# cts198859/deeprl_signal_control

Measured on AMD Instinct MI355X. Metric: env-steps/s (agents x envs x sim-steps/s), large_grid MA2C, higher is better.
Workload: dtype f32; 1 GPU; large_grid 5x5 (25 agents), MA2C LSTM policy (neighbour fingerprint gather), 1024 env instances per GPU; step = 120 control steps (x5 sim-steps) of every instance + 1 A2C update (BPTT, clip, RMSProp); envs_per_gpu=1024, n_step=120, agents=25, parallelism=env-sharded x1, live_vehicles=window mean over the timed region

## Files before the change

deeprl_signal_control_amd/csrc/tsc_model.hip:

```cpp
#include "tsc_common.h"
#include "tsc_gemm.h"
#include "../../include/tsc.h"

#include <cstdlib>
#include <type_traits>
#include <vector>

namespace {

using tsc::f32x16;
using tsc::f32x4;
using tsc::GemmArgs;

constexpr int kOut = 8;
constexpr int kL = 64;
constexpr int kG4 = 4 * kL;

struct Layout {
    int G, A, SMAX, AMAX, H;
    int NZ, fc;
    long long stride, oW1, ob1, oWx, oWh, obl, oWo, obo;
};

__device__ __forceinline__ float sigmoidf_(float x) {
// ... 103 lines not shown
            if (e < E) {
                const long long n = (long long)g * N + (long long)t * E + e;
                if (store) {
                    Z[n * kG4 + j] = ig; Z[n * kG4 + 64 + j] = fg; Z[n * kG4 + 128 + j] = og; Z[n * kG4 + 192 + j] = ug;
                    Cc[n * kL + j] = cn;
                }
                Hh[n * kL + j] = hn;
                if (t + 1 < T) keep = 1.0f - (float)done[(long long)(t + 1) * E + e];
                if (t + 1 == T && state_out) {
                    float *s = state_out + ((long long)g * E + e) * 2 * kL;
                    s[j] = cn; s[kL + j] = hn;
                }
            }
            c[r] = cn * keep;
            hs[j * kHsLd + erow[r]] = hn * keep;
        }
        __syncthreads();
    }
}

constexpr int kDz2Ld = kG4 + 4;
constexpr int kDh3Ld = kL + 4;

__global__ void __launch_bounds__(256, 2) lstm_bwd2_kernel(const float *__restrict__ params, Layout lay, float *Z,
                                                            const float *Cc, const float *state_bw, const float *dH,
                                                            const uint8_t *done, int T, int E) {
    extern __shared__ __attribute__((aligned(16))) char smem_raw[];
    float *dzs = (float *)smem_raw;
    float *dhs = dzs + 32 * kDz2Ld;
    const int g = blockIdx.x, e0 = blockIdx.y * 32;
    const int tid = threadIdx.x, lane = tid & 63, wave = tid >> 6, n = lane & 15, kq = lane >> 4;
    const int j = 16 * wave + n;
    const int er = tid >> 3, u0 = (tid & 7) * 8;
    const long long N = (long long)T * E;
    float bw[64];
    {
        const float4 *src = reinterpret_cast<const float4 *>(params + (long long)g * lay.stride + lay.oWh + (long long)j * kG4 + 4 * kq);
#pragma unroll
        for (int q = 0; q < 16; ++q) {
            const float4 w4 = src[4 * q];
            bw[4 * q] = w4.x; bw[4 * q + 1] = w4.y; bw[4 * q + 2] = w4.z; bw[4 * q + 3] = w4.w;
        }
    }
    float dc_rec[8];
#pragma unroll
    for (int r = 0; r < 8; ++r) dc_rec[r] = 0.f;
    const float *zg = Z + (long long)g * N * kG4, *cg = Cc + (long long)g * N * kL, *hg = dH + (long long)g * N * kL;
    const float *sg = state_bw + (long long)g * E * 2 * kL;
    const int e = e0 + er < E ? e0 + er : E - 1;
    const bool live = e0 + er < E;
    struct In { float4 gi[2], gf[2], go[2], gu[2], dhi[2], cpv[2]; float keep; };
    In in0, in1;
    float4 cc[2];
    auto request = [&](int t, In &o) {
        const long long nt = (long long)t * E;
        const float *zt = zg + nt * kG4, *ct = cg + nt * kL, *ht = hg + nt * kL;
        const float *cp_base = t > 0 ? ct - (long long)E * kL : sg;
        const unsigned cp_ld = t > 0 ? kL : 2 * kL;
        int zq = 0;
        asm volatile("" : "+v"(zq));
        const unsigned oz = (unsigned)((e + zq) * kG4 + u0) * 4u, oc = (unsigned)((e + zq) * kL + u0) * 4u;
#pragma unroll
        for (int a = 0; a < 2; ++a) {
            o.gi[a] = ldg((const float4 *)zt, oz + 16u * a); o.gf[a] = ldg((const float4 *)zt, oz + 256u + 16u * a);
            o.go[a] = ldg((const float4 *)zt, oz + 512u + 16u * a); o.gu[a] = ldg((const float4 *)zt, oz + 768u + 16u * a);
            o.dhi[a] = ldg((const float4 *)ht, oc + 16u * a);
            o.cpv[a] = ldg((const float4 *)cp_base, (unsigned)((e + zq) * cp_ld + u0) * 4u + 16u * a);
        }
        o.keep = done[nt + e] == 0 ? 1.0f : 0.0f;
    };
    {
        const float *ct = cg + (long long)(T - 1) * E * kL;
        cc[0] = ldg((const float4 *)ct, (unsigned)(e * kL + u0) * 4u); cc[1] = ldg((const float4 *)ct, (unsigned)(e * kL + u0) * 4u + 16u);
    }
    request(T - 1, in0);
    if (T > 1) request(T - 2, in1);
    float keep_next = 0.f;
    auto step = [&](int t, In &cur) {
        const long long nt = (long long)t * E;
        float *zw = Z + ((long long)g * N + nt) * kG4;
        const float keep = cur.keep;
        float4 dhr[2];
        if (t == T - 1) { dhr[0] = dhr[1] = make_float4(0.f, 0.f, 0.f, 0.f); }
        else {
            dhr[0] = *reinterpret_cast<const float4 *>(dhs + er * kDh3Ld + u0);
            dhr[1] = *reinterpret_cast<const float4 *>(dhs + er * kDh3Ld + u0 + 4);
        }
#pragma unroll
        for (int a = 0; a < 2; ++a) {
            const float igv[4] = {cur.gi[a].x, cur.gi[a].y, cur.gi[a].z, cur.gi[a].w}, fgv[4] = {cur.gf[a].x, cur.gf[a].y, cur.gf[a].z, cur.gf[a].w};
            const float ogv[4] = {cur.go[a].x, cur.go[a].y, cur.go[a].z, cur.go[a].w}, ugv[4] = {cur.gu[a].x, cur.gu[a].y, cur.gu[a].z, cur.gu[a].w};
            const float ccv[4] = {cc[a].x, cc[a].y, cc[a].z, cc[a].w}, cpw[4] = {cur.cpv[a].x, cur.cpv[a].y, cur.cpv[a].z, cur.cpv[a].w};
            const float dhv[4] = {cur.dhi[a].x, cur.dhi[a].y, cur.dhi[a].z, cur.dhi[a].w}, drv[4] = {dhr[a].x, dhr[a].y, dhr[a].z, dhr[a].w};
            float di[4], df[4], dg[4], du[4];
#pragma unroll
            for (int c = 0; c < 4; ++c) {
                const int r = 4 * a + c;
                const float ig = igv[c], fg = fgv[c], og = ogv[c], ug = ugv[c];
                const float cp = cpw[c] * keep;
                const float dh = dhv[c] + (keep_next != 0.f ? drv[c] : 0.f);
                const float tc = tanhf_(ccv[c]);
                dg[c] = dh * tc * og * (1.0f - og);
                const float dc = dh * og * (1.0f - tc * tc) + dc_rec[r];
                di[c] = dc * ug * ig * (1.0f - ig);
                df[c] = dc * cp * fg * (1.0f - fg);
                du[c] = dc * ig * (1.0f - ug * ug);
                dc_rec[r] = dc * fg * keep;
            }
            const float4 o_di = make_float4(di[0], di[1], di[2], di[3]), o_df = make_float4(df[0], df[1], df[2], df[3]);
            const float4 o_do = make_float4(dg[0], dg[1], dg[2], dg[3]), o_du = make_float4(du[0], du[1], du[2], du[3]);
            if (live) {
                const unsigned oz = (unsigned)((e0 + er) * kG4 + u0 + 4 * a) * 4u;
                stg((float4 *)zw, oz, o_di); stg((float4 *)zw, oz + 256u, o_df);
                stg((float4 *)zw, oz + 512u, o_do); stg((float4 *)zw, oz + 768u, o_du);
            }
            float *row = dzs + er * kDz2Ld + u0 + 4 * a;
// ... 13 lines not shown
        for (int q = 0; q < 16; ++q) {
            const float4 na = Aa[4 * (q + 1 < 16 ? q + 1 : q)], nb = Ab[4 * (q + 1 < 16 ? q + 1 : q)];
            acc[0] = __builtin_amdgcn_mfma_f32_16x16x4f32(pa.x, bw[4 * q], acc[0], 0, 0, 0);
            acc[1] = __builtin_amdgcn_mfma_f32_16x16x4f32(pb.x, bw[4 * q], acc[1], 0, 0, 0);
            acc[0] = __builtin_amdgcn_mfma_f32_16x16x4f32(pa.y, bw[4 * q + 1], acc[0], 0, 0, 0);
            acc[1] = __builtin_amdgcn_mfma_f32_16x16x4f32(pb.y, bw[4 * q + 1], acc[1], 0, 0, 0);
            acc[0] = __builtin_amdgcn_mfma_f32_16x16x4f32(pa.z, bw[4 * q + 2], acc[0], 0, 0, 0);
            acc[1] = __builtin_amdgcn_mfma_f32_16x16x4f32(pb.z, bw[4 * q + 2], acc[1], 0, 0, 0);
            acc[0] = __builtin_amdgcn_mfma_f32_16x16x4f32(pa.w, bw[4 * q + 3], acc[0], 0, 0, 0);
            acc[1] = __builtin_amdgcn_mfma_f32_16x16x4f32(pb.w, bw[4 * q + 3], acc[1], 0, 0, 0);
            pa = na; pb = nb;
            __builtin_amdgcn_sched_barrier(0);
        }
#pragma unroll
        for (int rt = 0; rt < 2; ++rt)
#pragma unroll
            for (int i = 0; i < 4; ++i) dhs[(16 * rt + 4 * kq + i) * kDh3Ld + j] = acc[rt][i];
        __syncthreads();
    };
    for (int t = T - 1; t >= 0; t -= 2) {
        step(t, in0);
        if (t >= 1) step(t - 1, in1);
    }
}

__device__ __forceinline__ void head_eval(const float *__restrict__ params, const Layout &lay, int a, int na,
                                          const float *hp, const float *hv, float *pi, float &v) {
    const float *Wo = params + (long long)(2 * a) * lay.stride + lay.oWo;
    const float *bo = params + (long long)(2 * a) * lay.stride + lay.obo;
    const float *Wv = params + (long long)(2 * a + 1) * lay.stride + lay.oWo;
    const float *bv = params + (long long)(2 * a + 1) * lay.stride + lay.obo;
    float lg[kOut];
#pragma unroll
    for (int k = 0; k < kOut; ++k) lg[k] = 0.f;
    float vv = 0.f;
    for (int jj = 0; jj < kL; ++jj) {
        const float h = hp[jj];
#pragma unroll
        for (int k = 0; k < kOut; ++k) lg[k] += h * Wo[jj * kOut + k];
        vv += hv[jj] * Wv[jj * kOut];
    }
    float mx = -INFINITY;
#pragma unroll
    for (int k = 0; k < kOut; ++k) { lg[k] += bo[k]; if (k < na && lg[k] > mx) mx = lg[k]; }
    float sum = 0.f;
#pragma unroll
// ... 20 lines not shown
        if (r < rows_left)
            *reinterpret_cast<float4 *>(dst + (long long)r * kL + c) = make_float4(t[r][c], t[r][c + 1], t[r][c + 2], t[r][c + 3]);
    }
}

__global__ void __launch_bounds__(64) head_fwd_kernel(const float *__restrict__ params, Layout lay, const int *n_act,
                                                      const float *Hh, int E, float *pi_out, float *v_out) {
    __shared__ float sp[64][kTLd], sv[64][kTLd];
    const int a = blockIdx.y, lane = threadIdx.x;
    const long long n0 = (long long)blockIdx.x * 64, left = E - n0;
    tile_load(Hh + ((long long)(2 * a) * E + n0) * kL, left, sp, lane);
    tile_load(Hh + ((long long)(2 * a + 1) * E + n0) * kL, left, sv, lane);
    __syncthreads();
    if (lane >= left) return;
    float pi[kOut], v;
    head_eval(params, lay, a, n_act[a], sp[lane], sv[lane], pi, v);
    const long long idx = (n0 + lane) * lay.A + a;
    for (int k = 0; k < lay.AMAX; ++k) pi_out[idx * lay.AMAX + k] = k < kOut ? pi[k] : 0.f;
    v_out[idx] = v;
}

constexpr int kHbPer = kL * kOut + kOut + kL + 1;

__global__ void __launch_bounds__(256, 3)
head_bwd2_kernel(const float *__restrict__ params, Layout lay, const int *__restrict__ n_act, const float *__restrict__ Hh,
                 const int *__restrict__ act, const float *__restrict__ Rs, const float *__restrict__ Advs, long long N,
                 long long rows_per_slice, float v_coef, float beta, float *__restrict__ dH, float *__restrict__ part,
                 double *stats) {
    __shared__ float red[4][16][36];
    const int a = blockIdx.y, sp = blockIdx.x, na = n_act[a];
    const int tid = threadIdx.x, c = tid & 15, grp = tid >> 4;
    const float *Pp = params + (long long)(2 * a) * lay.stride, *Pv = params + (long long)(2 * a + 1) * lay.stride;
    float wo[4][kOut], wv[4], bo[kOut];
#pragma unroll
    for (int u = 0; u < 4; ++u) {
#pragma unroll
        for (int k = 0; k < kOut; ++k) wo[u][k] = Pp[lay.oWo + (4 * c + u) * kOut + k];
        wv[u] = Pv[lay.oWo + (4 * c + u) * kOut];
    }
#pragma unroll
    for (int k = 0; k < kOut; ++k) bo[k] = Pp[lay.obo + k];
    const float bv = Pv[lay.obo];
    float aw[4][kOut], awv[4], ab[kOut], abv = 0.f;
#pragma unroll
    for (int u = 0; u < 4; ++u) {
        awv[u] = 0.f;
#pragma unroll
        for (int k = 0; k < kOut; ++k) aw[u][k] = 0.f;
    }
#pragma unroll
    for (int k = 0; k < kOut; ++k) ab[k] = 0.f;
    float lp = 0.f, lv = 0.f, le = 0.f;
    const long long n0 = (long long)sp * rows_per_slice;
    long long n1 = n0 + rows_per_slice;
    if (n1 > N) n1 = N;
    const float *hp = Hh + (long long)(2 * a) * N * kL + 4 * c, *hq = Hh + (long long)(2 * a + 1) * N * kL + 4 * c;
    float *dp = dH + (long long)(2 * a) * N * kL + 4 * c, *dq = dH + (long long)(2 * a + 1) * N * kL + 4 * c;
    const float invN = 1.0f / (float)N;
    for (long long nb = n0; nb < n1; nb += 16) {
        const long long n = nb + grp;
        const bool in = n < n1;
        const long long nc = in ? n : n1 - 1;
        const float4 h4 = *reinterpret_cast<const float4 *>(hp + nc * kL);
        const float4 g4 = *reinterpret_cast<const float4 *>(hq + nc * kL);
        const long long idx = nc * lay.A + a;
        const int ac = act[idx];
        const float adv = Advs[idx], R = Rs[idx];
        const float hh[4] = {h4.x, h4.y, h4.z, h4.w}, gg[4] = {g4.x, g4.y, g4.z, g4.w};
        float lg[kOut], vv = 0.f;
#pragma unroll
        for (int k = 0; k < kOut; ++k) lg[k] = 0.f;
#pragma unroll
        for (int u = 0; u < 4; ++u) {
#pragma unroll
            for (int k = 0; k < kOut; ++k) lg[k] += hh[u] * wo[u][k];
            vv += gg[u] * wv[u];
        }
#pragma unroll
        for (int o = 1; o < 16; o <<= 1) {
#pragma unroll
// ... 12 lines not shown
        const float pk = valid ? expf(lgm - mx) : 0.f;
        float sum = pk;
#pragma unroll
        for (int o = 1; o < 8; o <<= 1) sum += __shfl_xor(sum, o, 64);
        const float pim = pk / sum;
        const bool inr = pim >= 1e-10f;
        const float logpm = valid ? logf(fminf(fmaxf(pim, 1e-10f), 1.0f)) : 0.f;
        float gpi = 0.f;
        if (valid) {
            if (km == ac && inr) gpi += -adv * invN / fmaxf(pim, 1e-10f);
            gpi += beta * invN * (logpm + (inr ? 1.0f : 0.f));
        }
        float dot = pim * gpi, ent = valid ? -pim * logpm : 0.f, lpa = (km == (ac < na ? ac : 0)) ? logpm : 0.f;
#pragma unroll
        for (int o = 1; o < 8; o <<= 1) {
            dot += __shfl_xor(dot, o, 64); ent += __shfl_xor(ent, o, 64); lpa += __shfl_xor(lpa, o, 64);
        }
        const float dlm = (in && valid) ? pim * (gpi - dot) : 0.f;
        float dl[kOut];
        const int row0 = (tid & 63) & ~15;
#pragma unroll
        for (int k = 0; k < kOut; ++k) dl[k] = __shfl(dlm, row0 + k, 64);
        const float dv = in ? v_coef * (v - R) * invN : 0.f;
        float o4[4], q4[4];
#pragma unroll
        for (int u = 0; u < 4; ++u) {
            float sacc = 0.f;
#pragma unroll
            for (int k = 0; k < kOut; ++k) { sacc += dl[k] * wo[u][k]; aw[u][k] += hh[u] * dl[k]; }
            o4[u] = (lay.fc && !(hh[u] > 0.f)) ? 0.f : sacc;
            q4[u] = (lay.fc && !(gg[u] > 0.f)) ? 0.f : dv * wv[u];
            awv[u] += gg[u] * dv;
        }
        if (in) {
            *reinterpret_cast<float4 *>(dp + n * kL) = make_float4(o4[0], o4[1], o4[2], o4[3]);
            *reinterpret_cast<float4 *>(dq + n * kL) = make_float4(q4[0], q4[1], q4[2], q4[3]);
        }
        if (c == 0) {
#pragma unroll
            for (int k = 0; k < kOut; ++k) ab[k] += dl[k];
            abv += dv;
            if (in) {
                lp += -lpa * adv * invN;
                lv += 0.5f * v_coef * (R - v) * (R - v) * invN;
                le += -beta * ent * invN;
            }
        }
    }
    const int wave = tid >> 6;
#pragma unroll
    for (int o = 16; o < 64; o <<= 1) {
#pragma unroll
        for (int u = 0; u < 4; ++u) {
#pragma unroll
            for (int k = 0; k < kOut; ++k) aw[u][k] += __shfl_xor(aw[u][k], o, 64);
            awv[u] += __shfl_xor(awv[u], o, 64);
        }
#pragma unroll
        for (int k = 0; k < kOut; ++k) ab[k] += __shfl_xor(ab[k], o, 64);
// ... 20 lines not shown
    float *out = part + ((long long)sp * lay.A + a) * kHbPer;
    for (int j = tid; j < kHbPer; j += 256) {
        float acc = 0.f;
        if (j < kL * kOut) {
            const int jj = j / kOut, k = j % kOut;
            for (int w = 0; w < 4; ++w) acc += red[w][jj >> 2][(jj & 3) * kOut + k];
        } else if (j < kL * kOut + kOut) {
            for (int w = 0; w < 4; ++w) acc += redb[w][j - kL * kOut];
        } else if (j < kL * kOut + kOut + kL) {
            const int jj = j - (kL * kOut + kOut);
            for (int w = 0; w < 4; ++w) acc += red[w][jj >> 2][32 + (jj & 3)];
        } else {
            for (int w = 0; w < 4; ++w) acc += redb[w][kOut];
        }
        out[j] = acc;
    }
    if (stats && tid == 0) {
        double a0 = 0, a1 = 0, a2 = 0;
        for (int w = 0; w < 4; ++w) { a0 += redl[w][0]; a1 += redl[w][1]; a2 += redl[w][2]; }
        atomicAdd(&stats[a * 4 + 0], a0); atomicAdd(&stats[a * 4 + 1], a1); atomicAdd(&stats[a * 4 + 2], a2);
    }
}

__global__ void __launch_bounds__(256, 3)
head_bwd_ppo_kernel(const float *__restrict__ params, Layout lay, const int *__restrict__ n_act, const float *__restrict__ Hh,
                    const int *__restrict__ act, const float *__restrict__ Rs, const float *__restrict__ Advs, long long N,
                    long long rows_per_slice, float v_coef, float beta, float *__restrict__ dH, float *__restrict__ part,
                    double *stats, float *__restrict__ logp_old, int record, float clip_eps, double *ppo_stats) {
    __shared__ float red[4][16][36];
    const int a = blockIdx.y, sp = blockIdx.x, na = n_act[a];
    const int tid = threadIdx.x, c = tid & 15, grp = tid >> 4;
    const float *Pp = params + (long long)(2 * a) * lay.stride, *Pv = params + (long long)(2 * a + 1) * lay.stride;
    float wo[4][kOut], wv[4], bo[kOut];
#pragma unroll
    for (int u = 0; u < 4; ++u) {
#pragma unroll
        for (int k = 0; k < kOut; ++k) wo[u][k] = Pp[lay.oWo + (4 * c + u) * kOut + k];
        wv[u] = Pv[lay.oWo + (4 * c + u) * kOut];
    }
#pragma unroll
    for (int k = 0; k < kOut; ++k) bo[k] = Pp[lay.obo + k];
    const float bv = Pv[lay.obo];
    float aw[4][kOut], awv[4], ab[kOut], abv = 0.f;
#pragma unroll
    for (int u = 0; u < 4; ++u) {
        awv[u] = 0.f;
#pragma unroll
        for (int k = 0; k < kOut; ++k) aw[u][k] = 0.f;
    }
#pragma unroll
    for (int k = 0; k < kOut; ++k) ab[k] = 0.f;
    float lp = 0.f, lv = 0.f, le = 0.f, lc = 0.f, lk = 0.f;
    const long long n0 = (long long)sp * rows_per_slice;
    long long n1 = n0 + rows_per_slice;
    if (n1 > N) n1 = N;
    const float *hp = Hh + (long long)(2 * a) * N * kL + 4 * c, *hq = Hh + (long long)(2 * a + 1) * N * kL + 4 * c;
    float *dp = dH + (long long)(2 * a) * N * kL + 4 * c, *dq = dH + (long long)(2 * a + 1) * N * kL + 4 * c;
    const float invN = 1.0f / (float)N;
    for (long long nb = n0; nb < n1; nb += 16) {
        const long long n = nb + grp;
        const bool in = n < n1;
        const long long nc = in ? n : n1 - 1;
        const float4 h4 = *reinterpret_cast<const float4 *>(hp + nc * kL);
        const float4 g4 = *reinterpret_cast<const float4 *>(hq + nc * kL);
        const long long idx = nc * lay.A + a;
        const int ac = act[idx];
        const float adv = Advs[idx], R = Rs[idx];
        const float hh[4] = {h4.x, h4.y, h4.z, h4.w}, gg[4] = {g4.x, g4.y, g4.z, g4.w};
        float lg[kOut], vv = 0.f;
#pragma unroll
        for (int k = 0; k < kOut; ++k) lg[k] = 0.f;
#pragma unroll
        for (int u = 0; u < 4; ++u) {
#pragma unroll
            for (int k = 0; k < kOut; ++k) lg[k] += hh[u] * wo[u][k];
            vv += gg[u] * wv[u];
        }
#pragma unroll
        for (int o = 1; o < 16; o <<= 1) {
#pragma unroll
// ... 19 lines not shown
        float gpi = 0.f;
        float lpa = (km == (ac < na ? ac : 0)) ? logpm : 0.f;
#pragma unroll
        for (int o = 1; o < 8; o <<= 1) lpa += __shfl_xor(lpa, o, 64);
        const float lpo = record ? lpa : logp_old[idx];
        const float ratio = expf(lpa - lpo);
        const bool clipped = (adv > 0.f && ratio > 1.0f + clip_eps) || (adv < 0.f && ratio < 1.0f - clip_eps);
        if (record && in && c == 0) logp_old[idx] = lpa;
        if (valid) {
            if (km == ac && inr && !clipped) gpi += -adv * ratio * invN / fmaxf(pim, 1e-10f);
            gpi += beta * invN * (logpm + (inr ? 1.0f : 0.f));
        }
        float dot = pim * gpi, ent = valid ? -pim * logpm : 0.f;
#pragma unroll
        for (int o = 1; o < 8; o <<= 1) {
            dot += __shfl_xor(dot, o, 64); ent += __shfl_xor(ent, o, 64);
        }
        const float dlm = (in && valid) ? pim * (gpi - dot) : 0.f;
        float dl[kOut];
        const int row0 = (tid & 63) & ~15;
#pragma unroll
        for (int k = 0; k < kOut; ++k) dl[k] = __shfl(dlm, row0 + k, 64);
        const float dv = in ? v_coef * (v - R) * invN : 0.f;
        float o4[4], q4[4];
#pragma unroll
        for (int u = 0; u < 4; ++u) {
            float sacc = 0.f;
#pragma unroll
            for (int k = 0; k < kOut; ++k) { sacc += dl[k] * wo[u][k]; aw[u][k] += hh[u] * dl[k]; }
            o4[u] = (lay.fc && !(hh[u] > 0.f)) ? 0.f : sacc;
            q4[u] = (lay.fc && !(gg[u] > 0.f)) ? 0.f : dv * wv[u];
            awv[u] += gg[u] * dv;
        }
        if (in) {
            *reinterpret_cast<float4 *>(dp + n * kL) = make_float4(o4[0], o4[1], o4[2], o4[3]);
            *reinterpret_cast<float4 *>(dq + n * kL) = make_float4(q4[0], q4[1], q4[2], q4[3]);
        }
        if (c == 0) {
#pragma unroll
            for (int k = 0; k < kOut; ++k) ab[k] += dl[k];
            abv += dv;
            if (in) {
                const float rc = fminf(fmaxf(ratio, 1.0f - clip_eps), 1.0f + clip_eps);
                lp += -fminf(ratio * adv, rc * adv) * invN;
                lc += clipped ? invN : 0.f;
                lk += (lpo - lpa) * invN;
                lv += 0.5f * v_coef * (R - v) * (R - v) * invN;
                le += -beta * ent * invN;
            }
        }
    }
    const int wave = tid >> 6;
#pragma unroll
    for (int o = 16; o < 64; o <<= 1) {
#pragma unroll
        for (int u = 0; u < 4; ++u) {
#pragma unroll
            for (int k = 0; k < kOut; ++k) aw[u][k] += __shfl_xor(aw[u][k], o, 64);
            awv[u] += __shfl_xor(awv[u], o, 64);
// ... 1662 lines not shown
}

namespace {

constexpr size_t kLdsMax = 160 * 1024;

template <int... W, class F> bool with_width(int H, F &&f) { return ((H == W && (f(std::integral_constant<int, W>{}), true)) || ...); }
template <class F> bool with_fused_width(int H, F &&f) { return with_width<128, 160, 192, 224>(H, f); }

enum class Fwd : int8_t {
    Dense,
    Tile,
    Ws,
    FcThread,
    FcMfma
};
inline bool fills_cache(Fwd f) { return f == Fwd::Tile || f == Fwd::Ws || f == Fwd::FcMfma; }

struct Plan {
    Fwd fwd;
    bool dwxh;
    bool dx1w1;
    bool fc_bwd;
    int s_fwd;
    int s_upd;
};

}

struct tsc_model {
    Layout lay;
    Plan plan;
    int E, T, device;
    double gamma, rnorm, rclip, vcoef, max_norm, alpha, eps;
    hipStream_t stream;
    tsc::DeviceBufs bufs;
    int *n_act;
    int16_t *rowrange;
    int *wgmap; unsigned fwd_wgs;
    int dbg_tid;
    int *ftmask;
    int *krange;
    float *params, *grads, *ms, *WxT;
    float *Wg;
    int wg_dirty;
    float *state_fw, *state_bw;
    float *r_obs; int *r_act; double *r_rew; float *r_val; uint8_t *r_done;
    float *Rs, *Advs;
    float *logp_old;
    int ppo_ready;
    float *X1, *Z, *Hh, *Cc, *Hp, *dHh;
    double *norm2, *stats, *norm_part;
    float *ws, *wsc;
    size_t ws_floats, wsc_floats;
    size_t lds_fwd, lds_fused, lds_ws;
    int inplace;
    int cached_next;
    long long *dbg;
    long long nparam;
};

namespace {

int gemm(tsc_model *m, int kid, bool tn, int epi, int groups, int M, int N, int K, const float *A, long long sA, int lda,
         int gdivA, const float *B, long long sB, int ldb, float *C, long long sC, int ldc, const float *bias,
         long long sBias, const float *aux, long long sAux, int ldaux, const int16_t *rr, long long sRR,
         float *colsum, long long sColsum) {
    GemmArgs a;
    a.A = A; a.B = B; a.C = C; a.bias = bias; a.aux = aux; a.rr = rr; a.colsum = colsum;
    a.sA = sA; a.sB = sB; a.sC = sC; a.sBias = sBias; a.sAux = sAux; a.sRR = sRR; a.sColsum = sColsum;
    a.lda = lda; a.ldb = ldb; a.ldc = ldc; a.ldaux = ldaux; a.M = M; a.N = N; a.K = K; a.gdivA = gdivA;
    tsc::plan_splitk(a, groups, tn ? m->ws : nullptr, m->wsc, m->ws_floats, m->wsc_floats);
    tsc::ProfScope ps(kid, m->stream);
    tsc::launch_gemm_dyn(tn, epi, a, groups, m->stream);
// ... 73 lines not shown
        std::vector<int> fm((size_t)L.A * ncu, 0);
        for (int a = 0; a < L.A; ++a)
            for (int u = 0; u < ncu; ++u)
                for (int j = 0; j < L.SMAX && j < 64; ++j) {
                    const int lo = rr[((size_t)a * L.SMAX + j) * 2], hi = rr[((size_t)a * L.SMAX + j) * 2 + 1];
                    if (lo < 16 * u + 16 && hi > 16 * u) fm[(size_t)a * ncu + u] |= 1 << (j >> 4);
                }
        TSC_HIP(m->bufs.upload(&m->ftmask, fm.data(), fm.size()));
    }
    TSC_HIP(m->bufs.upload(&m->n_act, cfg->n_act, L.A));
    const long long E = n_env, T = m->T, N = E * T, G = L.G, A = L.A;
    TSC_HIP(m->bufs.alloc(&m->params, m->nparam, true)); TSC_HIP(m->bufs.alloc(&m->grads, m->nparam, true)); TSC_HIP(m->bufs.alloc(&m->ms, m->nparam, true));
    TSC_HIP(m->bufs.alloc(&m->WxT, G * L.H * kG4, true));
    TSC_HIP(m->bufs.alloc(&m->Wg, G * (L.H + kL) * kG4, true));
    m->wg_dirty = 1;
    TSC_HIP(m->bufs.alloc(&m->state_fw, G * E * 2 * kL, true)); TSC_HIP(m->bufs.alloc(&m->state_bw, G * E * 2 * kL, true));
    TSC_HIP(m->bufs.alloc(&m->r_obs, (N + E) * A * L.SMAX, true));
    TSC_HIP(m->bufs.alloc(&m->r_act, N * A, true)); TSC_HIP(m->bufs.alloc(&m->r_rew, N * A, true));
    TSC_HIP(m->bufs.alloc(&m->r_val, N * A, true)); TSC_HIP(m->bufs.alloc(&m->r_done, (T + 1) * E, true));
    TSC_HIP(m->bufs.alloc(&m->Rs, N * A, true)); TSC_HIP(m->bufs.alloc(&m->Advs, N * A, true));
    TSC_HIP(m->bufs.alloc(&m->X1, G * N * L.H + 32 * L.H, true));
    TSC_HIP(m->bufs.alloc(&m->Z, G * N * kG4, true));
    TSC_HIP(m->bufs.alloc(&m->Hh, G * N * kL, true)); TSC_HIP(m->bufs.alloc(&m->Cc, G * N * kL, true)); TSC_HIP(m->bufs.alloc(&m->Hp, G * N * kL, true));
    TSC_HIP(m->bufs.alloc(&m->dHh, G * N * kL, true));
    TSC_HIP(m->bufs.alloc(&m->norm2, A, true)); TSC_HIP(m->bufs.alloc(&m->stats, A * 6, true));
    TSC_HIP(m->bufs.alloc(&m->norm_part, A * kNormParts, true));
    m->logp_old = nullptr; m->ppo_ready = 0;
    m->ws_floats = (size_t)48 << 20; m->wsc_floats = (size_t)1 << 20;
    TSC_HIP(m->bufs.alloc(&m->ws, m->ws_floats, true)); TSC_HIP(m->bufs.alloc(&m->wsc, m->wsc_floats, true));
    m->lds_fwd = sizeof(float) * (64 * kWhLd + 64 * kHsLd);
    m->lds_fused = sizeof(float) * ((size_t)(L.H + 64) * kXLd + kL * kOut + kOut + 8);
    m->lds_ws = sizeof(float) * ((size_t)32 * (L.H + 64 + 4) + 64 * kWsLdx + (size_t)kL * kWsLdg + (size_t)kG4 * kWsLdg + 528 + (kWsBuf + 2) * 32 * kOut + (size_t)L.SMAX * L.H);
    m->dbg = nullptr;
    m->cached_next = 0;
    m->inplace = 0;

    const auto env_int = [](const char *name, int unset) { const char *ev = getenv(name); return ev ? atoi(ev) : unset; };
    const char *fwd_ws = getenv("TSC_FWD_WS");
    const bool unfused_dx = env_int("TSC_UNFUSED_DX", 0) != 0;
    m->dbg_tid = env_int("TSC_DBG_THREAD", 0);
    Plan &P = m->plan;
    P.s_upd = 256 / (int)G;
    if (P.s_upd < 1) P.s_upd = 1;
    P.s_fwd = P.s_upd < (E + 31) / 32 ? P.s_upd : (int)((E + 31) / 32);
    const bool wide = with_fused_width(L.H, [](auto) {}), narrow_obs = L.SMAX <= 64;
    const auto ws_fits = [&](long long per_split) { return (size_t)(P.s_upd * G * per_split) <= m->ws_floats; };
    if (!L.fc) {
        const bool tile = L.H % 32 == 0 && narrow_obs && m->lds_fused <= kLdsMax;
        P.fwd = !tile ? Fwd::Dense : wide && m->lds_ws <= kLdsMax && !(fwd_ws && fwd_ws[0] == '0') ? Fwd::Ws : Fwd::Tile;
        size_t lds_dwxh = 0;
        with_fused_width(L.H, [&](auto w) { lds_dwxh = dwxh_lds<(decltype(w)::value + kL) / 32>(); });
        P.dwxh = wide && lds_dwxh <= kLdsMax && !env_int("TSC_UNFUSED_DW", 0) && ws_fits((long long)(L.H + kL + 1) * kG4);
        P.dx1w1 = wide && narrow_obs && !unfused_dx && ws_fits((long long)2 * 65 * L.H);
    } else {
        P.fwd = wide && narrow_obs && env_int("TSC_FC_MFMA", 1) ? Fwd::FcMfma
              : L.H % 16 == 0 && narrow_obs && fc_thread_lds(L.H) <= kLdsMax ? Fwd::FcThread : Fwd::Dense;
        P.fc_bwd = wide && narrow_obs && !unfused_dx && ws_fits((long long)2 * 65 * L.H + (long long)(L.H + 1) * kL);
    }
    m->fwd_wgs = (unsigned)(G * P.s_fwd);
    if (P.fwd == Fwd::Ws && env_int("TSC_FWD_XCD", 1) && P.s_fwd > 1 && P.s_fwd < 256) {
        const int S = P.s_fwd, cap = (L.G * S + 7) / 8;
        std::vector<int> tab((size_t)8 * cap, -1), used(8, 0);
        for (int gg = 0; gg < L.G; ++gg) {
            int left = S, spn = 0;
            while (left > 0) {
                int x = 0;
                for (int k = 1; k < 8; ++k) if (cap - used[k] > cap - used[x]) x = k;
                const int take = left < cap - used[x] ? left : cap - used[x];
                for (int q = 0; q < take; ++q) tab[(size_t)(used[x] + q) * 8 + x] = (gg << 8) | (spn + q);
                used[x] += take; spn += take; left -= take;
            }
        }
        TSC_HIP(m->bufs.upload(&m->wgmap, tab.data(), tab.size()));
        m->fwd_wgs = (unsigned)tab.size();
    }
    hipError_t attr = hipSuccess;
    const auto allow_lds = [&attr](const void *k) {
        if (attr == hipSuccess) attr = hipFuncSetAttribute(k, hipFuncAttributeMaxDynamicSharedMemorySize, (int)kLdsMax);
    };
    allow_lds((const void *)lstm_bwd2_kernel);
    allow_lds((const void *)lstm_fwd_kernel<true>);
    allow_lds((const void *)lstm_fwd_kernel<false>);
    if (P.fwd == Fwd::Tile) allow_lds((const void *)policy_fwd_fused_kernel);
    if (P.fwd == Fwd::FcThread) allow_lds((const void *)policy_fwd_fc_kernel);
    with_fused_width(L.H, [&](auto w) {
        constexpr int H = decltype(w)::value;
        if (P.fwd == Fwd::Ws) allow_lds((const void *)policy_fwd_ws_kernel<(H + kL) / 2>);
        if (P.fwd == Fwd::FcMfma) allow_lds((const void *)policy_fwd_fc_mfma_kernel<H / 32>);
        if (P.dwxh) allow_lds((const void *)dwxh_kernel<(H + kL) / 32>);
        if (P.dx1w1) allow_lds((const void *)dx1w1_kernel2<H / 16>);
        if (P.fc_bwd) allow_lds((const void *)fc_bwd_kernel<H / 16>);
    });
    TSC_HIP(attr);
    hipLaunchKernelGGL(fill_kernel, dim3((unsigned)((m->nparam + 255) / 256)), dim3(256), 0, 0, m->ms, m->nparam, 1.0f);
    TSC_HIP(hipDeviceSynchronize());
    *out = guard.release();
    return 0;
}

int tsc_model_destroy(tsc_model *m) {
    if (!m) return 0;
    (void)hipSetDevice(m->device);
    delete m;
// ... 187 lines not shown
    const Layout &L = m->lay;
    const long long E = m->E, A = L.A, no = E * A * L.SMAX;
    if (obs != m->r_obs + (size_t)t * no) m->inplace = 0;
    tsc::ProfScope ps5(tsc::KID_ADD_TRANS, m->stream);
    hipLaunchKernelGGL(add_transition_kernel, dim3((unsigned)((no + 255) / 256)), dim3(256), 0, m->stream, (int)E, (int)A,
                       L.SMAX, obs, done_pre, action, reward, value, done_post, m->r_obs + t * no,
                       m->r_act + t * E * A, m->r_rew + t * E * A, m->r_val + t * E * A, m->r_done + t * E,
                       m->r_done + (t + 1) * E);
    ps5.stop();
    TSC_HIP(hipGetLastError());
    return 0;
}

struct PpoArgs { double clip_eps, lambda; int epoch; };

static int launch_head_bwd(tsc_model *m, long long N, double beta, const PpoArgs *ppo) {
    const Layout &L = m->lay;
    hipStream_t st = m->stream;
    int S = (int)((8 * 256 + L.A - 1) / L.A);
    long long rps = (N + S - 1) / S;
    rps = (rps + 15) / 16 * 16;
    S = (int)((N + rps - 1) / rps);
    if ((size_t)((long long)S * L.A * kHbPer) > m->ws_floats) return tsc::fail("head_bwd: workspace too small");
    if (ppo) {
        tsc::ProfScope ps7(tsc::KID_HEAD_BWD_PPO, m->stream);
        hipLaunchKernelGGL(head_bwd_ppo_kernel, dim3((unsigned)S, (unsigned)L.A), dim3(256), 0, st, m->params, L, m->n_act, m->Hh, m->r_act,
                           m->Rs, m->Advs, N, rps, (float)m->vcoef, (float)beta, m->dHh, m->ws, m->stats, m->logp_old,
                           ppo->epoch == 0 ? 1 : 0, (float)ppo->clip_eps, m->stats + 4 * L.A);
    } else {
        tsc::ProfScope ps7(tsc::KID_HEAD_BWD, m->stream);
        hipLaunchKernelGGL(head_bwd2_kernel, dim3((unsigned)S, (unsigned)L.A), dim3(256), 0, st, m->params, L, m->n_act, m->Hh, m->r_act,
                           m->Rs, m->Advs, N, rps, (float)m->vcoef, (float)beta, m->dHh, m->ws, m->stats);
    }
    {
        tsc::ProfScope ps(tsc::KID_DWO_GEMM, m->stream);
        const int tot = L.A * 2 * (kL * kOut + kOut);
        hipLaunchKernelGGL(head_bwd2_reduce_kernel, dim3((tot + 255) / 256), dim3(256), 0, st, m->ws, L.A, S, m->grads, L);
    }
    return hipGetLastError() == hipSuccess ? 0 : 1;
}

int tsc_model_rollout_slot(tsc_model *m, int32_t t, void *ptrs[6]) {
    if (!m || !ptrs || t < 0 || t > m->T) return tsc::fail("tsc_model_rollout_slot: slot %d outside [0,%d]", t, m ? m->T : 0);
    const Layout &L = m->lay;
    const long long E = m->E, A = L.A, no = E * A * L.SMAX;
    const bool in = t < m->T;
    ptrs[0] = m->r_obs + t * no;
    ptrs[1] = in ? (void *)(m->r_act + t * E * A) : nullptr;
    ptrs[2] = in ? (void *)(m->r_val + t * E * A) : nullptr;
    ptrs[3] = in ? (void *)(m->r_rew + t * E * A) : nullptr;
    ptrs[4] = m->r_done + t * E;
    ptrs[5] = in ? (void *)(m->r_done + (t + 1) * E) : nullptr;
    return 0;
}
// ... 37 lines not shown
                tsc::ProfScope ps(tsc::KID_DW1_GEMM, m->stream);
                const long long tot = ((long long)(L.SMAX + 1) * L.H + (long long)(L.H + 1) * kL) * G;
                hipLaunchKernelGGL(fc_bwd_reduce_kernel, dim3((unsigned)((tot + 255) / 256)), dim3(256), 0, st, m->ws, (int)G, S, L.H, L.SMAX,
                                   m->rowrange, g, L.stride, L.oW1, L.ob1, L.oWx);
            }
            TSC_HIP(hipGetLastError());
            m->cached_next = 0;
            return 0;
        }
        if (gemm(m, tsc::KID_DWX_GEMM, true, tsc::EPI_NONE, (int)G, L.H, kL, (int)N, m->X1, N * L.H, L.H, 1, m->dHh, N * kL, kL, g + L.oWx,
                 L.stride, kL, nullptr, 0, nullptr, 0, 0, nullptr, 0, g + L.obl, L.stride)) return tsc::fail("gemm failed");
        if (gemm(m, tsc::KID_DX1_GEMM, false, tsc::EPI_MASK_POS, (int)G, (int)N, L.H, kL, m->dHh, N * kL, kL, 1, m->WxT, (long long)L.H * kL, L.H,
                 m->X1, N * L.H, L.H, nullptr, 0, m->X1, N * L.H, L.H, nullptr, 0, nullptr, 0)) return tsc::fail("gemm failed");
    } else {
    if (m->cached_next != (int)T) {
        if (dense_forward(m, m->r_obs, N, m->X1, m->Z)) return tsc::fail("gemm launch failed");
        tsc::ProfScope ps2(tsc::KID_LSTM_FWD, m->stream);
        hipLaunchKernelGGL(lstm_fwd_kernel<true>, dim3((unsigned)G, (unsigned)((E + 63) / 64)), dim3(256), m->lds_fwd, st, m->params, L,
                           m->Z, m->state_bw, (float *)nullptr, m->Hh, m->Cc, m->Hp, m->r_done, (int)T, (int)E, 1);
        ps2.stop();
    }
    if (launch_head_bwd(m, N, beta, ppo)) return tsc::fail("head_bwd failed");
    tsc::ProfScope ps8(tsc::KID_LSTM_BWD, m->stream);
    hipLaunchKernelGGL(lstm_bwd2_kernel, dim3((unsigned)G, (unsigned)((E + 31) / 32)), dim3(256), sizeof(float) * 32 * (kDz2Ld + kDh3Ld), st,
                       m->params, L, m->Z, m->Cc, m->state_bw, m->dHh, m->r_done, (int)T, (int)E);
    ps8.stop();
    tsc::ProfScope ps9(tsc::KID_TRANSPOSE, m->stream);
    hipLaunchKernelGGL(transpose_wx_kernel, dim3((unsigned)((G * L.H * kG4 + 255) / 256)), dim3(256), 0, st, m->params, L, m->WxT);
    ps9.stop();
    TSC_HIP(hipGetLastError());
    if (P.dwxh) {
        const long long per = (long long)(L.H + kL + 1) * kG4;
        long long rps = (N + S - 1) / S;
        rps += rps & 1;
        {
            tsc::ProfScope ps(tsc::KID_DWX_GEMM, m->stream);
            with_fused_width(L.H, [&](auto w) {
                constexpr int NT = (decltype(w)::value + kL) / 32;
                hipLaunchKernelGGL(dwxh_kernel<NT>, dim3((unsigned)(S * G)), dim3(512), dwxh_lds<NT>(), st, m->X1, m->Hp, m->Z, N, (int)G, S,
                                   rps, m->ws, m->dbg);
            });
        }
        {
            tsc::ProfScope ps(tsc::KID_DWH_GEMM, m->stream);
            hipLaunchKernelGGL(dwxh_reduce_kernel, dim3((unsigned)((per * G + 255) / 256)), dim3(256), 0, st, m->ws, (int)G, S, per, g,
                               L.stride, L.oWx);
        }
        TSC_HIP(hipGetLastError());
// ... 128 lines not shown
    const size_t n = (size_t)m->T * m->E * m->lay.A;
    TSC_HIP(hipStreamSynchronize(m->stream));
    TSC_HIP(hipMemcpy(Rs, m->Rs, sizeof(float) * n, hipMemcpyDeviceToHost));
    TSC_HIP(hipMemcpy(Advs, m->Advs, sizeof(float) * n, hipMemcpyDeviceToHost));
    return 0;
}

int tsc_model_debug_read(tsc_model *m, int32_t what, int32_t g, int64_t row0, int64_t nrows, float *out_host) {
    if (!m || !out_host || g < 0 || g >= m->lay.G || row0 < 0 || nrows < 0) return tsc::fail("tsc_model_debug_read: bad arguments");
    const long long N = (long long)m->T * m->E;
    if (row0 + nrows > N) return tsc::fail("tsc_model_debug_read: rows [%lld, %lld) outside [0, %lld)", (long long)row0, (long long)(row0 + nrows), N);
    const float *base = nullptr;
    long long w = 0;
    switch (what) {
        case 0: base = m->X1; w = m->lay.H; break;
        case 1: base = m->Z; w = kG4; break;
        case 2: base = m->Hh; w = kL; break;
        case 3: base = m->Cc; w = kL; break;
        case 4: base = m->Hp; w = kL; break;
        case 5: base = m->dHh; w = kL; break;
        default: return tsc::fail("tsc_model_debug_read: unknown buffer %d", what);
    }
    if (m->lay.fc && (what == 1 || what == 3 || what == 4)) return tsc::fail("tsc_model_debug_read: buffer %d is LSTM-only", what);
    TSC_HIP(hipStreamSynchronize(m->stream));
    TSC_HIP(hipMemcpy(out_host, base + ((long long)g * N + row0) * w, sizeof(float) * (size_t)(nrows * w), hipMemcpyDeviceToHost));
    return 0;
}

int tsc_gemm_grouped_f32(int32_t form, int32_t epi, int32_t groups, int32_t M, int32_t N, int32_t K, const float *A,
                         int64_t sA, int32_t lda, const float *B, int64_t sB, int32_t ldb, float *C, int64_t sC,
                         int32_t ldc, const float *bias, const float *aux, const int16_t *rowrange, float *colsum,
                         float *splitk_ws, int64_t ws_floats, float *splitk_wsc, int64_t wsc_floats, void *hip_stream) {
    GemmArgs a;
    a.A = A; a.B = B; a.C = C; a.bias = bias; a.aux = aux; a.rr = rowrange; a.colsum = colsum;
    a.sA = sA; a.sB = sB; a.sC = sC; a.sBias = N; a.sAux = (long long)M * ldc; a.sRR = M; a.sColsum = N;
    a.lda = lda; a.ldb = ldb; a.ldc = ldc; a.ldaux = ldc; a.M = M; a.N = N; a.K = K; a.gdivA = 1;
    tsc::plan_splitk(a, groups, form != 0 ? splitk_ws : nullptr, splitk_wsc, (size_t)ws_floats, (size_t)wsc_floats);
    tsc::launch_gemm_dyn(form != 0, epi, a, groups, (hipStream_t)hip_stream);
    TSC_HIP(hipGetLastError());
    return 0;
}

}
```

Before: 394.7 million env-steps/s.

## Store value-head dH as a scalar per row and expand in LSTM backward

The head backward kernels now write the value-network gradient as one scalar dv per row instead of a full 64-wide dH vector (dv times Wv). The LSTM backward kernel, templated per group parity, reloads this scalar and multiplies by the value head weights in registers. This removes most of the value-branch dH write and read traffic and shrinks the dH buffer. The cost is extra template instantiations, a small recompute in the LSTM backward, and a dH layout that debug reads can no longer expose by default.

```diff
diff --git a/deeprl_signal_control_amd/csrc/tsc_model.hip b/deeprl_signal_control_amd/csrc/tsc_model.hip
--- a/deeprl_signal_control_amd/csrc/tsc_model.hip
+++ b/deeprl_signal_control_amd/csrc/tsc_model.hip
@@ -149,9 +149,10 @@
 constexpr int kDz2Ld = kG4 + 4;
 constexpr int kDh3Ld = kL + 4;
 
-__global__ void __launch_bounds__(256, 2) lstm_bwd2_kernel(const float *__restrict__ params, Layout lay, float *Z,
-                                                            const float *Cc, const float *state_bw, const float *dH,
-                                                            const uint8_t *done, int T, int E) {
+template <bool kValue>
+__device__ __forceinline__ void lstm_bwd2_body(const float *__restrict__ params, const Layout &lay, float *Z, const float *Cc,
+                                               const float *state_bw, const float *hg, const uint8_t *done, int T, int E) {
+    constexpr bool value = kValue;
     extern __shared__ __attribute__((aligned(16))) char smem_raw[];
     float *dzs = (float *)smem_raw;
     float *dhs = dzs + 32 * kDz2Ld;
@@ -172,7 +173,10 @@
     float dc_rec[8];
 #pragma unroll
     for (int r = 0; r < 8; ++r) dc_rec[r] = 0.f;
-    const float *zg = Z + (long long)g * N * kG4, *cg = Cc + (long long)g * N * kL, *hg = dH + (long long)g * N * kL;
+    const float *zg = Z + (long long)g * N * kG4, *cg = Cc + (long long)g * N * kL;
+    float wv[8];
+#pragma unroll
+    for (int c = 0; c < 8; ++c) wv[c] = value ? params[(long long)g * lay.stride + lay.oWo + (u0 + c) * kOut] : 0.f;
     const float *sg = state_bw + (long long)g * E * 2 * kL;
     const int e = e0 + er < E ? e0 + er : E - 1;
     const bool live = e0 + er < E;
@@ -181,7 +185,7 @@
     float4 cc[2];
     auto request = [&](int t, In &o) {
         const long long nt = (long long)t * E;
-        const float *zt = zg + nt * kG4, *ct = cg + nt * kL, *ht = hg + nt * kL;
+        const float *zt = zg + nt * kG4, *ct = cg + nt * kL, *ht = hg + nt * (value ? 1 : kL);
         const float *cp_base = t > 0 ? ct - (long long)E * kL : sg;
         const unsigned cp_ld = t > 0 ? kL : 2 * kL;
         int zq = 0;
@@ -191,9 +195,10 @@
         for (int a = 0; a < 2; ++a) {
             o.gi[a] = ldg((const float4 *)zt, oz + 16u * a); o.gf[a] = ldg((const float4 *)zt, oz + 256u + 16u * a);
             o.go[a] = ldg((const float4 *)zt, oz + 512u + 16u * a); o.gu[a] = ldg((const float4 *)zt, oz + 768u + 16u * a);
-            o.dhi[a] = ldg((const float4 *)ht, oc + 16u * a);
+            if constexpr (!value) o.dhi[a] = ldg((const float4 *)ht, oc + 16u * a);
             o.cpv[a] = ldg((const float4 *)cp_base, (unsigned)((e + zq) * cp_ld + u0) * 4u + 16u * a);
         }
+        if constexpr (value) o.dhi[0].x = ldg(ht, (unsigned)(e + zq) * 4u);
         o.keep = done[nt + e] == 0 ? 1.0f : 0.0f;
     };
     {
@@ -218,7 +223,12 @@
             const float igv[4] = {cur.gi[a].x, cur.gi[a].y, cur.gi[a].z, cur.gi[a].w}, fgv[4] = {cur.gf[a].x, cur.gf[a].y, cur.gf[a].z, cur.gf[a].w};
             const float ogv[4] = {cur.go[a].x, cur.go[a].y, cur.go[a].z, cur.go[a].w}, ugv[4] = {cur.gu[a].x, cur.gu[a].y, cur.gu[a].z, cur.gu[a].w};
             const float ccv[4] = {cc[a].x, cc[a].y, cc[a].z, cc[a].w}, cpw[4] = {cur.cpv[a].x, cur.cpv[a].y, cur.cpv[a].z, cur.cpv[a].w};
-            const float dhv[4] = {cur.dhi[a].x, cur.dhi[a].y, cur.dhi[a].z, cur.dhi[a].w}, drv[4] = {dhr[a].x, dhr[a].y, dhr[a].z, dhr[a].w};
+            const float drv[4] = {dhr[a].x, dhr[a].y, dhr[a].z, dhr[a].w};
+            float dhv[4] = {cur.dhi[a].x, cur.dhi[a].y, cur.dhi[a].z, cur.dhi[a].w};
+            if constexpr (value) {
+#pragma unroll
+                for (int c = 0; c < 4; ++c) dhv[c] = cur.dhi[0].x * wv[4 * a + c];
+            }
             float di[4], df[4], dg[4], du[4];
 #pragma unroll
             for (int c = 0; c < 4; ++c) {
@@ -278,6 +288,16 @@
         step(t, in0);
         if (t >= 1) step(t - 1, in1);
     }
+}
+
+template <bool kRec>
+__global__ void __launch_bounds__(256, 2) lstm_bwd2_kernel(const float *__restrict__ params, Layout lay, float *Z,
+                                                            const float *Cc, const float *state_bw, const float *dH,
+                                                            const uint8_t *done, int T, int E) {
+    const long long g = blockIdx.x, N = (long long)T * E;
+    if constexpr (!kRec) lstm_bwd2_body<false>(params, lay, Z, Cc, state_bw, dH + g * N * kL, done, T, E);
+    else if (g & 1) lstm_bwd2_body<true>(params, lay, Z, Cc, state_bw, dH + (long long)lay.A * N * kL + (g >> 1) * N, done, T, E);
+    else lstm_bwd2_body<false>(params, lay, Z, Cc, state_bw, dH + (g >> 1) * N * kL, done, T, E);
 }
 
 __device__ __forceinline__ void head_eval(const float *__restrict__ params, const Layout &lay, int a, int na,
@@ -344,11 +364,12 @@
 
 constexpr int kHbPer = kL * kOut + kOut + kL + 1;
 
+template <bool kCompact>
 __global__ void __launch_bounds__(256, 3)
 head_bwd2_kernel(const float *__restrict__ params, Layout lay, const int *__restrict__ n_act, const float *__restrict__ Hh,
                  const int *__restrict__ act, const float *__restrict__ Rs, const float *__restrict__ Advs, long long N,
-                 long long rows_per_slice, float v_coef, float beta, float *__restrict__ dH, float *__restrict__ part,
-                 double *stats) {
+                 long long rows_per_slice, float v_coef, float beta, float *__restrict__ dH,
+                 float *__restrict__ part, double *stats) {
     __shared__ float red[4][16][36];
     const int a = blockIdx.y, sp = blockIdx.x, na = n_act[a];
     const int tid = threadIdx.x, c = tid & 15, grp = tid >> 4;
@@ -377,7 +398,8 @@
     long long n1 = n0 + rows_per_slice;
     if (n1 > N) n1 = N;
     const float *hp = Hh + (long long)(2 * a) * N * kL + 4 * c, *hq = Hh + (long long)(2 * a + 1) * N * kL + 4 * c;
-    float *dp = dH + (long long)(2 * a) * N * kL + 4 * c, *dq = dH + (long long)(2 * a + 1) * N * kL + 4 * c;
+    float *dp = dH + (long long)(kCompact ? a : 2 * a) * N * kL + 4 * c;
+    float *dq = kCompact ? dH + (long long)lay.A * N * kL + (long long)a * N : dH + (long long)(2 * a + 1) * N * kL + 4 * c;
     const float invN = 1.0f / (float)N;
     for (long long nb = n0; nb < n1; nb += 16) {
         const long long n = nb + grp;
@@ -436,6 +458,21 @@
 #pragma unroll
         for (int k = 0; k < kOut; ++k) dl[k] = __shfl(dlm, row0 + k, 64);
         const float dv = in ? v_coef * (v - R) * invN : 0.f;
+        if constexpr (kCompact) {
+            float o4[4];
+#pragma unroll
+            for (int u = 0; u < 4; ++u) {
+                float sacc = 0.f;
+#pragma unroll
+                for (int k = 0; k < kOut; ++k) { sacc += dl[k] * wo[u][k]; aw[u][k] += hh[u] * dl[k]; }
+                o4[u] = sacc;
+                awv[u] += gg[u] * dv;
+            }
+            if (in) {
+                *reinterpret_cast<float4 *>(dp + n * kL) = make_float4(o4[0], o4[1], o4[2], o4[3]);
+                if (c == 0) dq[n] = dv;
+            }
+        } else {
         float o4[4], q4[4];
 #pragma unroll
         for (int u = 0; u < 4; ++u) {
@@ -449,6 +486,7 @@
         if (in) {
             *reinterpret_cast<float4 *>(dp + n * kL) = make_float4(o4[0], o4[1], o4[2], o4[3]);
             *reinterpret_cast<float4 *>(dq + n * kL) = make_float4(q4[0], q4[1], q4[2], q4[3]);
+        }
         }
         if (c == 0) {
 #pragma unroll
@@ -515,11 +553,13 @@
     }
 }
 
+template <bool kCompact>
 __global__ void __launch_bounds__(256, 3)
 head_bwd_ppo_kernel(const float *__restrict__ params, Layout lay, const int *__restrict__ n_act, const float *__restrict__ Hh,
                     const int *__restrict__ act, const float *__restrict__ Rs, const float *__restrict__ Advs, long long N,
-                    long long rows_per_slice, float v_coef, float beta, float *__restrict__ dH, float *__restrict__ part,
-                    double *stats, float *__restrict__ logp_old, int record, float clip_eps, double *ppo_stats) {
+                    long long rows_per_slice, float v_coef, float beta, float *__restrict__ dH,
+                    float *__restrict__ part, double *stats, float *__restrict__ logp_old, int record, float clip_eps,
+                    double *ppo_stats) {
     __shared__ float red[4][16][36];
     const int a = blockIdx.y, sp = blockIdx.x, na = n_act[a];
     const int tid = threadIdx.x, c = tid & 15, grp = tid >> 4;
@@ -548,7 +588,8 @@
     long long n1 = n0 + rows_per_slice;
     if (n1 > N) n1 = N;
     const float *hp = Hh + (long long)(2 * a) * N * kL + 4 * c, *hq = Hh + (long long)(2 * a + 1) * N * kL + 4 * c;
-    float *dp = dH + (long long)(2 * a) * N * kL + 4 * c, *dq = dH + (long long)(2 * a + 1) * N * kL + 4 * c;
+    float *dp = dH + (long long)(kCompact ? a : 2 * a) * N * kL + 4 * c;
+    float *dq = kCompact ? dH + (long long)lay.A * N * kL + (long long)a * N : dH + (long long)(2 * a + 1) * N * kL + 4 * c;
     const float invN = 1.0f / (float)N;
     for (long long nb = n0; nb < n1; nb += 16) {
         const long long n = nb + grp;
@@ -614,6 +655,21 @@
 #pragma unroll
         for (int k = 0; k < kOut; ++k) dl[k] = __shfl(dlm, row0 + k, 64);
         const float dv = in ? v_coef * (v - R) * invN : 0.f;
+        if constexpr (kCompact) {
+            float o4[4];
+#pragma unroll
+            for (int u = 0; u < 4; ++u) {
+                float sacc = 0.f;
+#pragma unroll
+                for (int k = 0; k < kOut; ++k) { sacc += dl[k] * wo[u][k]; aw[u][k] += hh[u] * dl[k]; }
+                o4[u] = sacc;
+                awv[u] += gg[u] * dv;
+            }
+            if (in) {
+                *reinterpret_cast<float4 *>(dp + n * kL) = make_float4(o4[0], o4[1], o4[2], o4[3]);
+                if (c == 0) dq[n] = dv;
+            }
+        } else {
         float o4[4], q4[4];
 #pragma unroll
         for (int u = 0; u < 4; ++u) {
@@ -627,6 +683,7 @@
         if (in) {
             *reinterpret_cast<float4 *>(dp + n * kL) = make_float4(o4[0], o4[1], o4[2], o4[3]);
             *reinterpret_cast<float4 *>(dq + n * kL) = make_float4(q4[0], q4[1], q4[2], q4[3]);
+        }
         }
         if (c == 0) {
 #pragma unroll
@@ -2335,6 +2392,7 @@
     bool dwxh;
     bool dx1w1;
     bool fc_bwd;
+    bool head_dh;
     int s_fwd;
     int s_upd;
 };
@@ -2362,7 +2420,8 @@
     float *Rs, *Advs;
     float *logp_old;
     int ppo_ready;
-    float *X1, *Z, *Hh, *Cc, *Hp, *dHh;
+    float *X1, *Z, *Hh, *Cc, *Hp;
+    float *dHh;
     double *norm2, *stats, *norm_part;
     float *ws, *wsc;
     size_t ws_floats, wsc_floats;
@@ -2482,7 +2541,7 @@
     TSC_HIP(m->bufs.alloc(&m->X1, G * N * L.H + 32 * L.H, true));
     TSC_HIP(m->bufs.alloc(&m->Z, G * N * kG4, true));
     TSC_HIP(m->bufs.alloc(&m->Hh, G * N * kL, true)); TSC_HIP(m->bufs.alloc(&m->Cc, G * N * kL, true)); TSC_HIP(m->bufs.alloc(&m->Hp, G * N * kL, true));
-    TSC_HIP(m->bufs.alloc(&m->dHh, G * N * kL, true));
+    m->dHh = nullptr;
     TSC_HIP(m->bufs.alloc(&m->norm2, A, true)); TSC_HIP(m->bufs.alloc(&m->stats, A * 6, true));
     TSC_HIP(m->bufs.alloc(&m->norm_part, A * kNormParts, true));
     m->logp_old = nullptr; m->ppo_ready = 0;
@@ -2517,6 +2576,8 @@
               : L.H % 16 == 0 && narrow_obs && fc_thread_lds(L.H) <= kLdsMax ? Fwd::FcThread : Fwd::Dense;
         P.fc_bwd = wide && narrow_obs && !unfused_dx && ws_fits((long long)2 * 65 * L.H + (long long)(L.H + 1) * kL);
     }
+    P.head_dh = L.fc || env_int("TSC_HEAD_DH", 0) != 0;
+    TSC_HIP(m->bufs.alloc(&m->dHh, P.head_dh ? G * N * kL : A * N * (kL + 1), true));
     m->fwd_wgs = (unsigned)(G * P.s_fwd);
     if (P.fwd == Fwd::Ws && env_int("TSC_FWD_XCD", 1) && P.s_fwd > 1 && P.s_fwd < 256) {
         const int S = P.s_fwd, cap = (L.G * S + 7) / 8;
@@ -2538,7 +2599,7 @@
     const auto allow_lds = [&attr](const void *k) {
         if (attr == hipSuccess) attr = hipFuncSetAttribute(k, hipFuncAttributeMaxDynamicSharedMemorySize, (int)kLdsMax);
     };
-    allow_lds((const void *)lstm_bwd2_kernel);
+    allow_lds(P.head_dh ? (const void *)lstm_bwd2_kernel<false> : (const void *)lstm_bwd2_kernel<true>);
     allow_lds((const void *)lstm_fwd_kernel<true>);
     allow_lds((const void *)lstm_fwd_kernel<false>);
     if (P.fwd == Fwd::Tile) allow_lds((const void *)policy_fwd_fused_kernel);
@@ -2772,14 +2833,15 @@
     rps = (rps + 15) / 16 * 16;
     S = (int)((N + rps - 1) / rps);
     if ((size_t)((long long)S * L.A * kHbPer) > m->ws_floats) return tsc::fail("head_bwd: workspace too small");
+    const Plan &P = m->plan;
     if (ppo) {
         tsc::ProfScope ps7(tsc::KID_HEAD_BWD_PPO, m->stream);
-        hipLaunchKernelGGL(head_bwd_ppo_kernel, dim3((unsigned)S, (unsigned)L.A), dim3(256), 0, st, m->params, L, m->n_act, m->Hh, m->r_act,
+        hipLaunchKernelGGL(P.head_dh ? head_bwd_ppo_kernel<false> : head_bwd_ppo_kernel<true>, dim3((unsigned)S, (unsigned)L.A), dim3(256), 0, st, m->params, L, m->n_act, m->Hh, m->r_act,
                            m->Rs, m->Advs, N, rps, (float)m->vcoef, (float)beta, m->dHh, m->ws, m->stats, m->logp_old,
                            ppo->epoch == 0 ? 1 : 0, (float)ppo->clip_eps, m->stats + 4 * L.A);
     } else {
         tsc::ProfScope ps7(tsc::KID_HEAD_BWD, m->stream);
-        hipLaunchKernelGGL(head_bwd2_kernel, dim3((unsigned)S, (unsigned)L.A), dim3(256), 0, st, m->params, L, m->n_act, m->Hh, m->r_act,
+        hipLaunchKernelGGL(P.head_dh ? head_bwd2_kernel<false> : head_bwd2_kernel<true>, dim3((unsigned)S, (unsigned)L.A), dim3(256), 0, st, m->params, L, m->n_act, m->Hh, m->r_act,
                            m->Rs, m->Advs, N, rps, (float)m->vcoef, (float)beta, m->dHh, m->ws, m->stats);
     }
     {
@@ -2863,8 +2925,8 @@
     }
     if (launch_head_bwd(m, N, beta, ppo)) return tsc::fail("head_bwd failed");
     tsc::ProfScope ps8(tsc::KID_LSTM_BWD, m->stream);
-    hipLaunchKernelGGL(lstm_bwd2_kernel, dim3((unsigned)G, (unsigned)((E + 31) / 32)), dim3(256), sizeof(float) * 32 * (kDz2Ld + kDh3Ld), st,
-                       m->params, L, m->Z, m->Cc, m->state_bw, m->dHh, m->r_done, (int)T, (int)E);
+    hipLaunchKernelGGL(P.head_dh ? lstm_bwd2_kernel<false> : lstm_bwd2_kernel<true>, dim3((unsigned)G, (unsigned)((E + 31) / 32)), dim3(256),
+                       sizeof(float) * 32 * (kDz2Ld + kDh3Ld), st, m->params, L, m->Z, m->Cc, m->state_bw, m->dHh, m->r_done, (int)T, (int)E);
     ps8.stop();
     tsc::ProfScope ps9(tsc::KID_TRANSPOSE, m->stream);
     hipLaunchKernelGGL(transpose_wx_kernel, dim3((unsigned)((G * L.H * kG4 + 255) / 256)), dim3(256), 0, st, m->params, L, m->WxT);
@@ -3039,6 +3101,7 @@
         default: return tsc::fail("tsc_model_debug_read: unknown buffer %d", what);
     }
     if (m->lay.fc && (what == 1 || what == 3 || what == 4)) return tsc::fail("tsc_model_debug_read: buffer %d is LSTM-only", what);
+    if (what == 5 && !m->plan.head_dh) return tsc::fail("tsc_model_debug_read: dH [G][N][64] exists under policy = fc or TSC_HEAD_DH=1 only");
     TSC_HIP(hipStreamSynchronize(m->stream));
     TSC_HIP(hipMemcpy(out_host, base + ((long long)g * N + row0) * w, sizeof(float) * (size_t)(nrows * w), hipMemcpyDeviceToHost));
     return 0;
```

Result: no change. 395.8 million env-steps/s, median of 6 (+0.3%).
